# soedinglab/MMseqs2

Hardware: AMD Instinct MI355X
Metric: sw_gcells_per_s (higher is better)
Workload: dtype int16

## Files before the change

mmseqs2_amd/csrc/mmgpu_api.hip:

```cpp
#include <algorithm>
#include <atomic>
#include <thread>
#include <cmath>
#include <cstdio>
#include <cstring>
#include <numeric>
#include <string>
#include <vector>

#include "mmgpu_internal.h"

#include <chrono>

using namespace mmgpu;

namespace mmgpu {
thread_local std::string g_last_error;
}
using mmgpu::g_last_error;

extern "C" const char *mmgpu_last_error(void) { return g_last_error.c_str(); }

extern "C" int mmgpu_init(mmgpu_ctx **out, int device_id) {
    if (!out) return fail(MMGPU_ERR_ARG, "mmgpu_init: ctx is NULL");
// ... 477 lines not shown
        v.len = b->m_len.as<uint32_t>();
        v.n = (uint32_t)b->m_h_len.size();
        v.max_len = b->m_max_len;
        v.h_len = b->m_h_len.data();
    } else {
        v.res = c->db.res;
        v.off4 = c->db.off4;
        v.len = c->db.len;
        v.n = c->db.n;
        v.max_len = c->db.max_len;
        v.h_len = c->h_len.data();
    }
    return v;
}

static void pick_class(uint32_t qlen, int *rows_per_lane, bool *multi) {
    constexpr uint32_t max_rows = 16u * (uint32_t)SW_MAX_R;
    const uint32_t n_tiles = (qlen + max_rows - 1) / max_rows;
    const uint32_t rows = (qlen + n_tiles - 1) / n_tiles;
    *rows_per_lane = (int)std::max<uint32_t>(1u, (rows + 15) / 16);
    *multi = n_tiles > 1;
}

static uint32_t job_slots(uint32_t round, uint64_t rounds) {
    const uint64_t slots = std::max<uint64_t>(1, rounds) * round;
    if (slots >= JOB_ROUND) return (uint32_t)std::min<uint64_t>(JOB_HITS, slots / JOB_ROUND * JOB_ROUND);
    return slots >= 16 ? 16u : round;
}

struct DeviceLists {
    const mmgpu_pf_hit *hits = nullptr;
    const uint32_t *counts = nullptr;
// ... 276 lines not shown
    }
    if (multi && mode >= MMGPU_SW_START)
        add_rev_jobs(i, hit_cursor, pf_stride, shape, (uint64_t)Q.qlen * ((Q.qlen + c->mean_len) / 2 + 1));
    max_tlen = tv.max_len;
}

int SwPrepare::copy_queries() {
    for (uint32_t i = 0; i < nq; i++) {
        const mmgpu_sw_query &Q = qs[i];
        if (Q.qlen == 0) {
            b->h_qout_off[i + 1] = out_cursor;
            continue;
        }
        int qminp;
        if (int e = copy_query(i, &qminp)) return e;
        int rpl; bool multi;
        pick_class(Q.qlen, &rpl, &multi);
        any_multi |= multi;
        const uint32_t shape = (multi ? 32u : 0u) + (uint32_t)rpl - 1;
        const int grp = sw_shape_group(shape);
        const uint32_t held = multi && sw_multi_resident(sw_tiles(Q.qlen, rpl), rpl, par->alphabet, SW_RESIDENT_LDS) ? sw_tiles(Q.qlen, rpl) : 1u;
        b->group_lds[grp] = std::max(b->group_lds[grp], (size_t)held * sw_profile_bytes(rpl, par->alphabet));
        const uint32_t round = (multi && Q.qlen >= LONG_QUERY) ? JOB_ROUND / 4 : JOB_ROUND;
        const uint32_t n_slots = pf ? pf_stride : dense ? dense->count[i] : Q.n_targets;
        if (pf) add_slot_jobs(i, shape, round, multi);
        else deferred.push_back(Deferred{i, hit_cursor, out_cursor, shape, round, multi});
        hit_cursor += n_slots;
        out_cursor += n_slots;
        b->h_qout_off[i + 1] = out_cursor;
    }
    return MMGPU_OK;
}

void SwPrepare::cut_list_jobs_of(size_t from, size_t to) {
    std::vector<uint32_t> ord;
    for (size_t d = from; d < to; d++) {
        const Deferred &D = deferred[d];
        const mmgpu_sw_query &Q = qs[D.query];
// ... 493 lines not shown
            L.out = b->x_out ? b->x_out : b->d_out.as<mmgpu_sw_hit>();
            L.mat = b->d_mat.as<int8_t>();
            L.alphabet = b->alphabet;
            L.gap_open = b->gap_open;
            L.gap_extend = b->gap_extend;
            L.q_hit_count = b->from_pf ? b->d_pf_counts.as<uint32_t>() : nullptr;
            L.hit_stride = b->slot_stride;
            L.scratch = b->d_scratch.as<uint2>();
            L.scratch_cols = b->scratch_cols;
            L.scratch_busy = b->d_scratch_busy.as<uint32_t>();
            L.scratch_slots = std::max<uint32_t>(b->scratch_slots, 1);
            L.resident_lds = SW_RESIDENT_LDS;
            L.rev_mode = rev_only ? 2 : (b->mode == MMGPU_SW_START_NOT_WORD ? 1 : 0);
            L.rev_only = rev_only ? 1 : 0;
            L.rev_force = rev_force;
            HIP_TRY(launch_sw(L, g, b->group_lds[g], b->mode >= MMGPU_SW_START, st));
            if (g == SW_GROUPS - 1 && b->n_rev_jobs && b->mode >= MMGPU_SW_START) {
                SwLaunch Rv = L;
                Rv.jobs = b->d_jobs.as<SwJob>() + b->n_jobs;
                Rv.n_jobs = b->n_rev_jobs;
                HIP_TRY(launch_sw_rev_multi(Rv, b->group_lds[g], st));
            }
            if (getenv("MMGPU_TRACE")) {
                fprintf(stderr, "[sw_run] group %d jobs %u lds %zu both %d from_pf %d scratch_cols %u\n", g, L.n_jobs, b->group_lds[g], (int)(b->mode >= MMGPU_SW_START), (int)b->from_pf, b->scratch_cols);
                fflush(stderr);
                const auto t0 = std::chrono::steady_clock::now();
                hipError_t e = hipStreamSynchronize(st);
                fprintf(stderr, "[sw_run] group %d done after %.2f ms: %s\n", g,
                        std::chrono::duration<double, std::milli>(std::chrono::steady_clock::now() - t0).count(), hipGetErrorString(e));
                fflush(stderr);
// ... 774 lines not shown
```

mmseqs2_amd/csrc/mmgpu_internal.h:

```cpp
#ifndef MMGPU_INTERNAL_H
#define MMGPU_INTERNAL_H

#include <hip/hip_runtime.h>
#include <stdint.h>
#include <cstdlib>
#include <cstring>

#include <algorithm>
#include <array>
#include <string>
#include <map>
#include <mutex>
#include <chrono>
#include <memory>
#include <vector>
#include <thread>
#include <atomic>

#include "../../include/mmgpu.h"
#include "nucl_core.h"
#include "block_plan.h"

namespace mmgpu {

// ... 55 lines not shown
    const uint32_t *hit_out;
    mmgpu_sw_hit *out;
    const int8_t *mat;
    int alphabet;
    int gap_open, gap_extend;
    uint2 *scratch;
    uint32_t scratch_cols;
    uint32_t *scratch_busy;
    uint32_t scratch_slots;
    uint32_t resident_lds = 0;
    const uint32_t *q_hit_count;
    uint32_t hit_stride;
    int rev_mode = 0;
    int rev_only = 0;
    const uint8_t *rev_force = nullptr;
};

constexpr int SW_PF_MAX_LIST = 16384;
constexpr int SW_FROM_PF_STAT_SLOTS = 64;

struct SwFromPfArgs {
    const mmgpu_pf_hit *pf_hits;
    uint32_t pf_stride;
    const uint32_t *hit_count;
    uint32_t stride;
    const uint32_t *q_off;
    const uint32_t *t_len;
    uint32_t *hit_target, *hit_out;
    unsigned long long *cells, *pairs;
    uint32_t *count_copy;
// ... 21 lines not shown
static_assert(SW_GROUPS == 3 || SW_GROUPS == 4, "three or four kernel groups");
int sw_shape_group(uint32_t shape);
hipError_t launch_sw(const SwLaunch &L, int group, size_t lds_bytes, bool both_passes, hipStream_t stream);
#ifndef MMGPU_SW_HALF
#define MMGPU_SW_HALF 1
#endif
bool launch_sw_half(const SwLaunch &L, int group, size_t lds_bytes, bool both_passes, hipStream_t stream);
void warm_sw_half();

constexpr int SW_LDS_HEADER = SW_REV_JOB_MAX * 2 + 64;
__host__ __device__ constexpr int lane_stride_bytes(int R) {
    int slots = (R * 2 + 15) / 16;
    if ((slots & 1) == 0) slots += 1;
    return slots * 16;
}
__host__ __device__ constexpr uint32_t sw_profile_bytes(int R, int alphabet) {
    return (uint32_t)(alphabet + 1) * 16u * (uint32_t)lane_stride_bytes(R);
}
#ifndef MMGPU_SW_RESIDENT_LDS
#define MMGPU_SW_RESIDENT_LDS 65536
#endif
constexpr uint32_t SW_RESIDENT_LDS = MMGPU_SW_RESIDENT_LDS;
static_assert(SW_RESIDENT_LDS <= 65536u, "a workgroup asks for at most 64 KB of dynamic LDS");
__host__ __device__ constexpr uint32_t sw_tiles(uint32_t qlen, int R) { return (qlen + 16u * (uint32_t)R - 1u) / (16u * (uint32_t)R); }
__host__ __device__ constexpr bool sw_multi_resident(uint32_t n_tiles, int R, int alphabet, uint32_t budget) {
    return (unsigned long long)n_tiles * sw_profile_bytes(R, alphabet) + (unsigned long long)SW_LDS_HEADER <= (unsigned long long)budget;
}
static_assert(sw_multi_resident(2, 28, 21, 65536) && sw_multi_resident(3, 24, 21, 65536) && !sw_multi_resident(3, 25, 21, 65536) &&
              !sw_multi_resident(4, 22, 21, 65536) && !sw_multi_resident(2, 8, 21, 0), "residency rule");

constexpr int SCAN_CLASSES = 5;
constexpr int SCAN_MULTI = SCAN_CLASSES - 1;
constexpr int SCAN_MAX_R = 32;
constexpr int SCAN_ROUND = 32;
constexpr int SCAN_JOB_TARGETS = 16 * SCAN_ROUND;
__host__ __device__ constexpr int scan_class_rows(int cls) { return cls == 0 ? 8 : cls == 1 ? 16 : cls == 2 ? 24 : 32; }
__host__ __device__ constexpr uint32_t scan_cols(uint32_t len, int R) { return (len + (uint32_t)R - 1u) / (uint32_t)R * (uint32_t)R; }
__host__ __device__ constexpr uint32_t scan_park_row_words(uint32_t longest) { return 2u * ((scan_cols(longest, SCAN_MAX_R) + 1u + 15u) & ~15u); }

constexpr uint64_t SCAN_NO_PROFILE = ~0ull;

struct ScanJob {
    uint32_t query;
    uint32_t begin, end;
// ... 868 lines not shown
```

mmseqs2_amd/csrc/sw_body.h:

```cpp
#pragma once
#include "mmgpu_internal.h"
#include "pf_device.h"

namespace mmgpu {

namespace {

constexpr int GROUP = 16;
constexpr int WAVES = 4;
constexpr int GROUPS_PER_WAVE = 64 / GROUP;
constexpr int HITS_PER_WAVE = 2 * GROUPS_PER_WAVE;
constexpr unsigned NEG2 = 0x80008000u;

typedef short s16x2 __attribute__((ext_vector_type(2)));
typedef unsigned short u16x2 __attribute__((ext_vector_type(2)));

__device__ __forceinline__ unsigned pk_add_sat(unsigned a, unsigned b) {
    return __builtin_bit_cast(unsigned, __builtin_elementwise_add_sat(__builtin_bit_cast(s16x2, a),
                                                                      __builtin_bit_cast(s16x2, b)));
}
__device__ __forceinline__ unsigned pk_max_s(unsigned a, unsigned b) {
    return __builtin_bit_cast(unsigned, __builtin_elementwise_max(__builtin_bit_cast(s16x2, a),
                                                                  __builtin_bit_cast(s16x2, b)));
}
// ... 13 lines not shown
constexpr int SW_HALF_MAX_GAP = 2048;
constexpr int SW_HALF_MARK = -1;
typedef _Float16 h16x2 __attribute__((ext_vector_type(2)));
__device__ __forceinline__ h16x2 as_h(unsigned a) { return __builtin_bit_cast(h16x2, a); }
__device__ __forceinline__ unsigned as_u(h16x2 a) { return __builtin_bit_cast(unsigned, a); }
__device__ __forceinline__ unsigned h_add(unsigned a, unsigned b) { return as_u(as_h(a) + as_h(b)); }
__device__ __forceinline__ unsigned h_sub(unsigned a, unsigned b) { return as_u(as_h(a) - as_h(b)); }
__device__ __forceinline__ unsigned h_max(unsigned a, unsigned b) {
    return as_u(__builtin_elementwise_maximum(as_h(a), as_h(b)));
}
__device__ __forceinline__ unsigned h_max3(unsigned a, unsigned b, unsigned c) {
    return as_u(__builtin_elementwise_maximum(__builtin_elementwise_maximum(as_h(a), as_h(b)), as_h(c)));
}
__device__ __forceinline__ unsigned short h_bits(int v) { return __builtin_bit_cast(unsigned short, (_Float16)v); }
__device__ __forceinline__ int h_value(unsigned bits) { return (int)(float)__builtin_bit_cast(_Float16, (unsigned short)bits); }
__device__ __forceinline__ unsigned from_lane_above(unsigned head, unsigned v) {
    return __builtin_amdgcn_update_dpp(head, v, 0x111 , 0xF, 0xF, false);
}
__device__ __forceinline__ unsigned from_lane_above_or_zero(unsigned v) {
    return __builtin_amdgcn_update_dpp(0u, v, 0x111 , 0xF, 0xF, true);
}

#ifndef MMGPU_SW_PREFETCH
#define MMGPU_SW_PREFETCH 1
#endif
#define SW_KEEP_IN_ROW(x) asm volatile("" : "+v"(x))

template <int R>
struct Tile {
    static constexpr int ROWS = GROUP * R;
    static constexpr int LANE_STRIDE = lane_stride_bytes(R);
    static constexpr int ROW_STRIDE = GROUP * LANE_STRIDE;
};
static_assert(GROUP == 16, "sw_profile_bytes and sw_tiles (mmgpu_internal.h) assume 16-lane groups");

template <int R, bool REV, bool HALF = false>
__device__ __forceinline__ void build_profile(unsigned char *lds, const uint8_t *q, const int8_t *cb, int qlen,
                                              int tile_base, const int8_t *mat, int alphabet, const int8_t *prof) {
    using T = Tile<R>;
    const int total = (alphabet + 1) * T::ROWS;
    for (int idx = threadIdx.x; idx < total; idx += blockDim.x) {
        const int letter = idx / T::ROWS;
        const int row = idx - letter * T::ROWS;
        const int rg = tile_base + row;
        short v = (short)-32768;
        if (letter < alphabet && rg < qlen) {
            const int qi = REV ? (qlen - 1 - rg) : rg;
            v = prof ? (short)prof[letter * qlen + qi] : (short)((int)mat[letter * alphabet + q[qi]] + (int)cb[qi]);
        }
        const int lane = row / R, r = row - lane * R;
        if constexpr (HALF) v = (short)h_bits(v);
        *reinterpret_cast<short *>(lds + letter * T::ROW_STRIDE + lane * T::LANE_STRIDE + r * 2) = v;
    }
}
// ... 2 lines not shown
    const mmgpu_sw_hit &f = L.out[slot];
    const int s = f.score;
    if (L.rev_mode == 2) return s > 0 && L.rev_force[slot] != 0;
    return s > 0 && s >= min_start && !(L.rev_mode == 1 && f.word != 0);
}

constexpr int SW_REV_JOB_HITS = 1024;
static_assert(SW_REV_JOB_HITS == SW_REV_JOB_MAX, "host and kernel disagree on the reverse job size");
static_assert(SW_LDS_HEADER == SW_REV_JOB_HITS * 2 + 64, "the header holds the live hits and the scheduling words");
constexpr int SW_HALF_FLAG_AT = SW_REV_JOB_HITS * 2 + 20;
__device__ __forceinline__ uint32_t sw_half_any_marked() {
    extern __shared__ __attribute__((aligned(16))) unsigned char lds_all[];
    return *reinterpret_cast<const uint32_t *>(lds_all + SW_HALF_FLAG_AT);
}

template <int R, bool MULTI, bool REV, bool PF, bool HALF = false, bool MARKED = false>
__device__ __forceinline__ void sw_body(const SwLaunch &L, const SwJob job) {
    static_assert(!(HALF || MARKED) || (!MULTI && !REV && !(HALF && MARKED)), "f16 and its int16 re-run: single-tile forward scans");
    constexpr bool PACKED = REV || MARKED;
    using T = Tile<R>;
    extern __shared__ __attribute__((aligned(16))) unsigned char lds_all[];
    uint16_t *live = reinterpret_cast<uint16_t *>(lds_all);
    uint32_t *live_wave = reinterpret_cast<uint32_t *>(lds_all + SW_REV_JOB_HITS * 2);
    uint32_t *next_chunk = reinterpret_cast<uint32_t *>(lds_all + SW_REV_JOB_HITS * 2 + 16);
    uint32_t *half_flag = reinterpret_cast<uint32_t *>(lds_all + SW_HALF_FLAG_AT);
    unsigned char *lds = lds_all + SW_LDS_HEADER;
    if (MULTI) __builtin_amdgcn_s_setprio(3);
    const int lane = threadIdx.x & 63;
    const int wave = __builtin_amdgcn_readfirstlane(threadIdx.x >> 6);
    const int g = lane & (GROUP - 1);
    const int grp = lane / GROUP;

    const uint32_t qbeg = L.q_off[job.query];
    const int qlen = (int)(L.q_off[job.query + 1] - qbeg);
    const uint8_t *q = L.q_res + qbeg;
    const int8_t *cb = L.q_cb + qbeg;
    const int qbias = L.q_bias[job.query];
    const int8_t *prof = nullptr;
    if (L.q_prof_off) {
        const uint32_t po = L.q_prof_off[job.query];
        if (po != 0xFFFFFFFFu) prof = L.q_prof + po;
    }
    const int n_tiles = MULTI ? (int)sw_tiles((uint32_t)qlen, R) : 1;
    const uint32_t tile_bytes = sw_profile_bytes(R, L.alphabet);
    const bool resident = MULTI && sw_multi_resident((uint32_t)n_tiles, R, L.alphabet, L.resident_lds);
    const bool dynamic = !MULTI || resident;
    auto build_all_tiles = [&]() {
        for (int tile = 0; tile < n_tiles; ++tile)
            build_profile<R, REV>(lds + (uint32_t)tile * tile_bytes, q, cb, qlen, tile * T::ROWS, L.mat, L.alphabet, prof);
        __syncthreads();
    };

    const unsigned go2 = (HALF ? (unsigned)h_bits(L.gap_open) : (unsigned)L.gap_open) * 0x10001u;
    const unsigned ge2 = (HALF ? (unsigned)h_bits(L.gap_extend) : (unsigned)L.gap_extend) * 0x10001u;
    const unsigned pad_letter = (unsigned)L.alphabet;

    if (threadIdx.x == 0) *next_chunk = 0;
    if (HALF && threadIdx.x == 0) *half_flag = 0;
    if (!MULTI && !PACKED) {
        build_profile<R, REV, HALF>(lds, q, cb, qlen, 0, L.mat, L.alphabet, prof);
        __syncthreads();
    }
    if (MULTI && !REV && resident) build_all_tiles();

    uint32_t n_hits = job.hit_end - job.hit_begin;
    if (PACKED) {
        const int min_start = REV ? L.q_minstart[job.query] : 0;
        uint32_t total = 0;
        for (uint32_t base = 0; base < n_hits; base += WAVES * 64) {
            const uint32_t idx = base + threadIdx.x;
            bool pass = false;
            if (idx < n_hits) {
                const uint32_t slot = L.hit_out[job.hit_begin + idx];
                pass = MARKED ? L.out[slot].score == SW_HALF_MARK : sw_rev_wanted(L, slot, min_start);
            }
// ... 2 lines not shown
            __syncthreads();
            uint32_t before = 0, round_total = 0;
#pragma unroll
            for (int w = 0; w < WAVES; ++w) {
                const uint32_t c = live_wave[w];
                before += w < wave ? c : 0u;
                round_total += c;
            }
            if (pass) live[total + before + (uint32_t)__popcll(bal & ((1ull << lane) - 1ull))] = (uint16_t)idx;
            total += round_total;
            __syncthreads();
        }
        n_hits = total;
        if (n_hits == 0) return;
        if (!MULTI) {
            build_profile<R, REV>(lds, q, cb, qlen, 0, L.mat, L.alphabet, prof);
            __syncthreads();
        }
        if (MULTI && resident) build_all_tiles();
    }
    const uint32_t n_iter = (n_hits + WAVES * HITS_PER_WAVE - 1) / (WAVES * HITS_PER_WAVE);

    for (uint32_t it = 0; dynamic || it < n_iter; ++it) {
        uint32_t chunk = it * WAVES + wave;
        if (dynamic) {
            if (lane == 0) chunk = atomicAdd(next_chunk, 1u);
            chunk = __builtin_amdgcn_readfirstlane(chunk);
        }
        const uint32_t slot0 = chunk * HITS_PER_WAVE;
        if (dynamic && slot0 >= n_hits) break;

// ... 14 lines not shown
            fb = fa;
            if (vA) fa = L.out[L.hit_out[hA]];
            if (vB) fb = L.out[L.hit_out[hB]];
            colsA = vA ? fa.t_end + 1 : 0;
            colsB = vB ? fb.t_end + 1 : 0;
            endA = colsA > 0 ? fa.t_end : 0;
            endB = colsB > 0 ? fb.t_end : 0;
            r0A = colsA > 0 ? qlen - 1 - fa.q_end : 0;
            r0B = colsB > 0 ? qlen - 1 - fb.q_end : 0;
            rev_target = (colsA > 0 ? (unsigned)fa.score & 0xFFFFu : 0xFFFFu) | ((colsB > 0 ? (unsigned)fb.score & 0xFFFFu : 0xFFFFu) << 16);
        }
        int ncols = colsA > colsB ? colsA : colsB;
        ncols = max(ncols, __shfl_xor(ncols, 16));
        ncols = max(ncols, __shfl_xor(ncols, 32));
        ncols = __builtin_amdgcn_readfirstlane(ncols);
        const int nsteps = ncols + GROUP - 1;
        int mincols = colsA < colsB ? colsA : colsB;
        mincols = min(mincols, __shfl_xor(mincols, 16));
        mincols = min(mincols, __shfl_xor(mincols, 32));
        mincols = __builtin_amdgcn_readfirstlane(mincols);

        unsigned long long bestA = 0, bestB = 0;

        uint2 *scr = nullptr;
        unsigned scr_grp = 0;
        if (MULTI) {
            scr = L.scratch + (size_t)((job.shape >> 8) * WAVES + wave) * GROUPS_PER_WAVE * 2 * L.scratch_cols;
            scr_grp = (unsigned)grp * 2u * L.scratch_cols;
        }

        for (int tile = 0; tile < n_tiles; ++tile) {
// ... 83 lines not shown
                    b = bfi(mb, b, pad4);
                }
                const unsigned lo = __builtin_amdgcn_perm(b, a, REV ? 0x06020703u : 0x05010400u);
                const unsigned hi = __builtin_amdgcn_perm(b, a, REV ? 0x04000501u : 0x07030602u);
                lq = ((unsigned long long)hi << 32) | lo;
            };
            auto head_letters = [&](int c, int j) -> unsigned {
                if (LETTER_BLOCKS && LETTER_QUEUE) { const unsigned v = (unsigned)lq; lq >>= 16; return v; }
                if (LETTER_BLOCKS) return (unsigned)(lq >> (16 * j));
                const unsigned sh = (unsigned)(REV ? 3 - j : j) * 8u;
                const unsigned la0 = __builtin_amdgcn_ubfe(wA, sh, 8u);
                const unsigned lb0 = __builtin_amdgcn_ubfe(wB, sh, 8u);
                return (c < colsA ? la0 : pad_letter) | ((c < colsB ? lb0 : pad_letter) << 8);
            };
            letter_block(0);
            let = from_lane_above(head_letters(0, 0), let);
            if (PF) load_rows(let, pav_next, pbv_next);

            for (int s0 = -1; s0 < nsteps; s0 += 4) {
            if (MULTI && s0 > 0 && ((s0 + 1) & 15) == 0) {
                bnd = bnd_next;
                if (has_above) bnd_next = boundary16(((s0 + 1) >> 4) + 1);
            }
            const int jn = min(4, nsteps - s0);
#pragma nounroll
            for (int j = s0 < 0 ? 1 : 0; j < jn; ++j) {
                const int s = s0 + j;
                if (has_below && s >= GROUP) {
                    if (g == GROUP - 1) (scr_out + (s - GROUP))[scr_grp] = make_uint2(out_H, out_F);
                }
                const unsigned Hup = MULTI ? from_lane_above(bnd.x, out_H) : from_lane_above_or_zero(out_H);
                unsigned f = MULTI ? from_lane_above(bnd.y, out_F) : from_lane_above_or_zero(out_F);
                if (MULTI) {
                    bnd.x = __builtin_amdgcn_update_dpp(bnd.x, bnd.x, 0x12F, 0xF, 0xF, false);
                    bnd.y = __builtin_amdgcn_update_dpp(bnd.y, bnd.y, 0x12F, 0xF, 0xF, false);
                }
                unsigned pav[ND], pbv[ND];
                if (PF) {
#pragma unroll
                    for (int k = 0; k < ND; ++k) { pav[k] = pav_next[k]; pbv[k] = pbv_next[k]; }
                } else {
                    load_rows(let, pav, pbv);
                }

                unsigned hd = Hup_prev;
                Hup_prev = Hup;
                unsigned cmax = 0;
                unsigned pre[R], es[R];
#pragma unroll
                for (int r = 0; r < R; ++r) {
                    unsigned P = __builtin_amdgcn_perm(pbv[r / 2], pav[r / 2], (r & 1) ? 0x07060302u : 0x05040100u);
                    if (REV) P = __builtin_amdgcn_bitop3_b32(aux[r], P, NEG2, 0xCA);
                    if constexpr (HALF) {
                        pre[r] = h_add(r == 0 ? hd : Hp[r - 1], P);
                        es[r] = h_sub(E[r], ge2);
                    } else {
                        pre[r] = pk_max_s(pk_add_sat(r == 0 ? hd : Hp[r - 1], P), E[r]);
                        es[r] = pk_sub_sat_u(E[r], ge2);
                    }
                }
                let = from_lane_above(head_letters(s + 1, j), let);
                if (PF) load_rows(let, pav_next, pbv_next);
#pragma unroll
                for (int r = 0; r < R; ++r) {
                    unsigned h;
                    if constexpr (HALF) {
                        h = h_max3(pre[r], E[r], f);
                        const unsigned fs = h_sub(f, ge2);
                        const unsigned t = h_sub(h, go2);
                        cmax = r == 0 ? h : h_max(cmax, h);
                        f = h_max3(fs, t, 0u);
                        E[r] = h_max3(es[r], t, 0u);
                    } else {
                        h = pk_max_s(pre[r], f);
                        const unsigned fs = pk_sub_sat_u(f, ge2);
                        const unsigned t = pk_sub_sat_u(h, go2);
// ... 49 lines not shown
            if (!REV) {
#pragma unroll
                for (int r = R - 1; r >= 0; --r) {
                    if ((aux[r] & 0xFFFFu) == sA) rowA_first = (unsigned)r;
                    if ((aux[r] >> 16) == sB) rowB_first = (unsigned)r;
                }
            } else {
                sA = sA == (rev_target & 0xFFFFu) ? sA : 0u;
                sB = sB == (rev_target >> 16) ? sB : 0u;
            }
            const unsigned rgA = (unsigned)(tile_base + g * R) + rowA_first;
            const unsigned rgB = (unsigned)(tile_base + g * R) + rowB_first;
            unsigned long long keyA = sA ? ((unsigned long long)sA << 32) | ((0xFFFFu - (bestcol & 0xFFFFu)) << 16) | (0xFFFFu - rgA) : 0ull;
            unsigned long long keyB = sB ? ((unsigned long long)sB << 32) | ((0xFFFFu - (bestcol >> 16)) << 16) | (0xFFFFu - rgB) : 0ull;
#pragma unroll
            for (int m = 1; m < GROUP; m <<= 1) {
                const unsigned long long oa = __shfl_xor(keyA, m), ob = __shfl_xor(keyB, m);
                keyA = oa > keyA ? oa : keyA;
                keyB = ob > keyB ? ob : keyB;
            }
            bestA = keyA > bestA ? keyA : bestA;
            bestB = keyB > bestB ? keyB : bestB;
        }

        if (g == 0) {
#pragma unroll
            for (int half = 0; half < 2; ++half) {
                const bool valid = half ? vB : vA;
                if (!valid) continue;
                const unsigned long long key = half ? bestB : bestA;
                const uint32_t h = half ? hB : hA;
// ... 13 lines not shown
                    *o = res;
                    if (marked) *half_flag = 1;
                } else {
                    const int end = half ? endB : endA;
                    const int cols = half ? colsB : colsA;
                    if (cols > 0) {
                        o->t_start = (score == o->score) ? end - col : -2;
                        o->q_start = (score == o->score) ? qlen - 1 - row : -2;
                    }
                }
            }
        }
    }
}

template <int R, bool MULTI, bool BOTH>
__device__ __forceinline__ void sw_passes(const SwLaunch &L, const SwJob &job) {
    if constexpr (R <= SW_MAX_R) {
        constexpr bool PF = MMGPU_SW_PREFETCH && !MULTI && (BOTH || R <= 24);
        if (!(BOTH && L.rev_only)) sw_body<R, MULTI, false, PF>(L, job);
        if constexpr (BOTH && !MULTI) {
            __threadfence_block();
            __syncthreads();
            sw_body<R, MULTI, true, PF>(L, job);
        }
    }
}

#ifndef MMGPU_SW_WAVES_G0F
#define MMGPU_SW_WAVES_G0F 4
#endif
#ifndef MMGPU_SW_WAVES_G0B
#define MMGPU_SW_WAVES_G0B 2
#endif
#ifndef MMGPU_SW_WAVES_G1F
#define MMGPU_SW_WAVES_G1F 3
#endif
#ifndef MMGPU_SW_WAVES_G1B
#define MMGPU_SW_WAVES_G1B 2
// ... 6 lines not shown
```

mmseqs2_amd/csrc/sw_half_kernel.hip:

```cpp
#include "mmgpu_internal.h"
#include "pf_device.h"
#include "sw_body.h"

namespace mmgpu {

namespace {

template <int R, bool BOTH>
__device__ __forceinline__ void sw_half_passes(const SwLaunch &L, const SwJob &job) {
    if constexpr (R <= SW_MAX_R) {
        constexpr bool PF = MMGPU_SW_PREFETCH && (BOTH || R <= 24);
        sw_body<R, false, false, PF, true, false>(L, job);
        __threadfence_block();
        __syncthreads();
        if (sw_half_any_marked()) {
            sw_body<R, false, false, PF, false, true>(L, job);
            __threadfence_block();
            __syncthreads();
        }
        if constexpr (BOTH) sw_body<R, false, true, PF>(L, job);
    }
}

constexpr bool SW_HALF_FORWARD_ONLY[3] = {false, false, false};

template <int G, bool BOTH>
__global__ __launch_bounds__(WAVES * 64)
__attribute__((amdgpu_waves_per_eu(G == 0 ? (BOTH ? MMGPU_SW_WAVES_G0B : MMGPU_SW_WAVES_G0F)
                                           : (G == 1 ? (BOTH ? MMGPU_SW_WAVES_G1B : MMGPU_SW_WAVES_G1F) : SW_MIN_WAVES),
                                   G == 1 && BOTH ? MMGPU_SW_WAVES_G1B : 8))) void sw_half_kernel(SwLaunch L) {
    SwJob job = L.jobs[blockIdx.x];
    if (L.q_hit_count) {
        const uint32_t lim = job.query * L.hit_stride + L.q_hit_count[job.query];
        job.hit_end = job.hit_end < lim ? job.hit_end : lim;
        if (job.hit_end <= job.hit_begin) return;
    }
#define MMGPU_SW_SINGLE(R) case (R) - 1: sw_half_passes<R, BOTH>(L, job); break;
    if constexpr (G == 0) {
        switch (job.shape & 0xFFu) {
            MMGPU_SW_SINGLE(1) MMGPU_SW_SINGLE(2) MMGPU_SW_SINGLE(3) MMGPU_SW_SINGLE(4) MMGPU_SW_SINGLE(5) MMGPU_SW_SINGLE(6)
            MMGPU_SW_SINGLE(7) MMGPU_SW_SINGLE(8) MMGPU_SW_SINGLE(9) MMGPU_SW_SINGLE(10) MMGPU_SW_SINGLE(11) MMGPU_SW_SINGLE(12)
            default: break;
        }
    } else if constexpr (G == 1) {
        switch (job.shape & 0xFFu) {
            MMGPU_SW_SINGLE(13) MMGPU_SW_SINGLE(14) MMGPU_SW_SINGLE(15) MMGPU_SW_SINGLE(16) MMGPU_SW_SINGLE(17) MMGPU_SW_SINGLE(18)
            MMGPU_SW_SINGLE(19) MMGPU_SW_SINGLE(20) MMGPU_SW_SINGLE(21) MMGPU_SW_SINGLE(22) MMGPU_SW_SINGLE(23) MMGPU_SW_SINGLE(24)
            default: break;
        }
    } else {
        switch (job.shape & 0xFFu) {
            MMGPU_SW_SINGLE(25) MMGPU_SW_SINGLE(26) MMGPU_SW_SINGLE(27) MMGPU_SW_SINGLE(28) MMGPU_SW_SINGLE(29) MMGPU_SW_SINGLE(30)
            MMGPU_SW_SINGLE(31) MMGPU_SW_SINGLE(32)
            default: break;
        }
    }
#undef MMGPU_SW_SINGLE
}

#ifdef MMGPU_SW_HALF_AUDIT_FORWARD
template __global__ void sw_half_kernel<0, false>(SwLaunch);
template __global__ void sw_half_kernel<1, false>(SwLaunch);
template __global__ void sw_half_kernel<2, false>(SwLaunch);
#endif

}

bool launch_sw_half(const SwLaunch &L, int group, size_t lds_bytes, bool both_passes, hipStream_t stream) {
    if (group < 0 || group > 2 || (group == 2 && SW_GROUPS != 4)) return false;
    if (!both_passes && !SW_HALF_FORWARD_ONLY[group]) return false;
    dim3 grid(L.n_jobs), block(WAVES * 64);
    const size_t lds = lds_bytes + SW_LDS_HEADER;
// ... 15 lines not shown
```

mmseqs2_amd/csrc/sw_kernel.hip:

```cpp
#include "mmgpu_internal.h"
#include "pf_device.h"
#include "sw_body.h"

namespace mmgpu {

namespace {

#define MMGPU_SW_MULTI_ALL                                                                                                          \
    MMGPU_SW_MULTI(8) MMGPU_SW_MULTI(9) MMGPU_SW_MULTI(10) MMGPU_SW_MULTI(11) MMGPU_SW_MULTI(12) MMGPU_SW_MULTI(13) MMGPU_SW_MULTI(14) \
    MMGPU_SW_MULTI(15) MMGPU_SW_MULTI(16) MMGPU_SW_MULTI(17) MMGPU_SW_MULTI(18) MMGPU_SW_MULTI(19) MMGPU_SW_MULTI(20) MMGPU_SW_MULTI(21) \
    MMGPU_SW_MULTI(22) MMGPU_SW_MULTI(23) MMGPU_SW_MULTI(24) MMGPU_SW_MULTI(25) MMGPU_SW_MULTI(26) MMGPU_SW_MULTI(27) MMGPU_SW_MULTI(28) \
    MMGPU_SW_MULTI(29) MMGPU_SW_MULTI(30) MMGPU_SW_MULTI(31) MMGPU_SW_MULTI(32)
template <int G, bool BOTH>
__global__ __launch_bounds__(WAVES * 64)
__attribute__((amdgpu_waves_per_eu(G == 0 ? (BOTH ? MMGPU_SW_WAVES_G0B : MMGPU_SW_WAVES_G0F)
                                           : (G == 1 ? (BOTH ? MMGPU_SW_WAVES_G1B : MMGPU_SW_WAVES_G1F) : SW_MIN_WAVES),
                                   G == 1 && BOTH ? MMGPU_SW_WAVES_G1B : 8))) void sw_kernel(SwLaunch L) {
    SwJob job = L.jobs[blockIdx.x];
    if (L.q_hit_count) {
        const uint32_t lim = job.query * L.hit_stride + L.q_hit_count[job.query];
        job.hit_end = job.hit_end < lim ? job.hit_end : lim;
        if (job.hit_end <= job.hit_begin) return;
    }
    __shared__ uint32_t scratch_slot;
    const bool claims = G == SW_GROUPS - 1 && (job.shape & 0xFFu) >= 32u;
    if (claims) {
        if (threadIdx.x == 0) {
            uint32_t s = blockIdx.x % L.scratch_slots;
            while (atomicCAS(&L.scratch_busy[s], 0u, 1u) != 0u) s = s + 1 == L.scratch_slots ? 0u : s + 1;
            scratch_slot = s;
        }
        __syncthreads();
        job.shape = (job.shape & 0xFFu) | (scratch_slot << 8);
    }
#define MMGPU_SW_SINGLE(R) case (R) - 1: sw_passes<R, false, BOTH>(L, job); break;
#define MMGPU_SW_MULTI(R) case 32 + (R) - 1: sw_passes<R, true, BOTH>(L, job); break;
    if constexpr (G == 0) {
        switch (job.shape & 0xFFu) {
            MMGPU_SW_SINGLE(1) MMGPU_SW_SINGLE(2) MMGPU_SW_SINGLE(3) MMGPU_SW_SINGLE(4) MMGPU_SW_SINGLE(5) MMGPU_SW_SINGLE(6)
            MMGPU_SW_SINGLE(7) MMGPU_SW_SINGLE(8) MMGPU_SW_SINGLE(9) MMGPU_SW_SINGLE(10) MMGPU_SW_SINGLE(11) MMGPU_SW_SINGLE(12)
            default: break;
        }
    } else if constexpr (G == 1) {
        switch (job.shape & 0xFFu) {
            MMGPU_SW_SINGLE(13) MMGPU_SW_SINGLE(14) MMGPU_SW_SINGLE(15) MMGPU_SW_SINGLE(16) MMGPU_SW_SINGLE(17) MMGPU_SW_SINGLE(18)
            MMGPU_SW_SINGLE(19) MMGPU_SW_SINGLE(20) MMGPU_SW_SINGLE(21) MMGPU_SW_SINGLE(22) MMGPU_SW_SINGLE(23) MMGPU_SW_SINGLE(24)
            default: break;
        }
    } else if constexpr (SW_GROUPS == 4 && G == 2) {
        switch (job.shape & 0xFFu) {
            MMGPU_SW_SINGLE(25) MMGPU_SW_SINGLE(26) MMGPU_SW_SINGLE(27) MMGPU_SW_SINGLE(28) MMGPU_SW_SINGLE(29) MMGPU_SW_SINGLE(30)
            MMGPU_SW_SINGLE(31) MMGPU_SW_SINGLE(32)
            default: break;
        }
    } else if constexpr (SW_GROUPS == 4) {
        switch (job.shape & 0xFFu) {
            MMGPU_SW_MULTI_ALL
            default: break;
        }
    } else {
        switch (job.shape & 0xFFu) {
            MMGPU_SW_SINGLE(25) MMGPU_SW_SINGLE(26) MMGPU_SW_SINGLE(27) MMGPU_SW_SINGLE(28) MMGPU_SW_SINGLE(29) MMGPU_SW_SINGLE(30)
            MMGPU_SW_SINGLE(31) MMGPU_SW_SINGLE(32)
            MMGPU_SW_MULTI_ALL
            default: break;
        }
    }
#undef MMGPU_SW_SINGLE
#undef MMGPU_SW_MULTI
#undef MMGPU_SW_MULTI_ALL
    if (claims) {
        __syncthreads();
        if (threadIdx.x == 0) {
            __threadfence();
            atomicExch(&L.scratch_busy[scratch_slot], 0u);
        }
    }
}

__global__ __launch_bounds__(WAVES * 64) __attribute__((amdgpu_waves_per_eu(SW_MIN_WAVES))) void sw_rev_multi_kernel(SwLaunch L) {
    SwJob job = L.jobs[blockIdx.x];
    if (L.q_hit_count) {
        const uint32_t lim = job.query * L.hit_stride + L.q_hit_count[job.query];
        job.hit_end = job.hit_end < lim ? job.hit_end : lim;
        if (job.hit_end <= job.hit_begin) return;
// ... 100 lines not shown
        int rev = 0;
        if (hipOccupancyMaxActiveBlocksPerMultiprocessor(&rev, sw_rev_multi_kernel, WAVES * 64, lds) == hipSuccess) per_cu = std::max(per_cu, rev);
    }
    if (e != hipSuccess || per_cu < 1) per_cu = 8;
    per_cu = per_cu + 1 > 8 ? 8 : per_cu + 1;
    return (uint32_t)per_cu * (uint32_t)(compute_units > 0 ? compute_units : 256);
}

hipError_t launch_sw_rev_multi(const SwLaunch &L, size_t lds_bytes, hipStream_t stream) {
    if (L.n_jobs == 0) return hipSuccess;
    hipLaunchKernelGGL(sw_rev_multi_kernel, dim3(L.n_jobs), dim3(WAVES * 64), lds_bytes + SW_LDS_HEADER, stream, L);
    return hipGetLastError();
}

int sw_shape_group(uint32_t shape) {
    if (shape >= 32) return SW_GROUPS - 1;
    const int R = (int)shape + 1;
    return R <= 12 ? 0 : (R <= 24 ? 1 : 2);
}

static bool sw_half_eligible(const SwLaunch &L) {
    return MMGPU_SW_HALF && !L.rev_only && L.gap_open >= 0 && L.gap_open <= SW_HALF_MAX_GAP && L.gap_extend >= 0 &&
           L.gap_extend <= SW_HALF_MAX_GAP;
}

hipError_t launch_sw(const SwLaunch &L, int group, size_t lds_bytes, bool both_passes, hipStream_t stream) {
    static_assert(GROUP == 16, "the shape codes assume 16-lane groups");
    if (L.n_jobs == 0) return hipSuccess;
    if (sw_half_eligible(L) && launch_sw_half(L, group, lds_bytes, both_passes, stream)) return hipGetLastError();
    dim3 grid(L.n_jobs), block(WAVES * 64);
    const size_t lds = lds_bytes + SW_LDS_HEADER;
    switch (group * 2 + (both_passes ? 1 : 0)) {
        case 0: hipLaunchKernelGGL((sw_kernel<0, false>), grid, block, lds, stream, L); break;
        case 1: hipLaunchKernelGGL((sw_kernel<0, true>), grid, block, lds, stream, L); break;
        case 2: hipLaunchKernelGGL((sw_kernel<1, false>), grid, block, lds, stream, L); break;
        case 3: hipLaunchKernelGGL((sw_kernel<1, true>), grid, block, lds, stream, L); break;
        case 4: hipLaunchKernelGGL((sw_kernel<2, false>), grid, block, lds, stream, L); break;
        case 5: hipLaunchKernelGGL((sw_kernel<2, true>), grid, block, lds, stream, L); break;
        case 6: hipLaunchKernelGGL((sw_kernel<SW_GROUPS - 1, false>), grid, block, lds, stream, L); break;
        case 7: hipLaunchKernelGGL((sw_kernel<SW_GROUPS - 1, true>), grid, block, lds, stream, L); break;
        default: return hipErrorInvalidValue;
    }
// ... 11 lines not shown
```

Baseline: 4913.

## Add 32-lane wide single-tile SW shape for queries up to twice max tile

Queries longer than one 16-lane tile but at most twice that length now go to a new wide shape. It uses 32-lane groups spanning two DPP rows, so the whole query sits in one tile. This avoids the multi-tile path with its scratch boundary exchange, scratch slot claiming and repeated passes over targets. The cost is an extra cross-row DPP per lane shift, twice the profile LDS, half the hits per wave, and a smaller job round. A half-precision path is also wired in behind an env switch.

```diff
diff --git a/mmseqs2_amd/csrc/mmgpu_api.hip b/mmseqs2_amd/csrc/mmgpu_api.hip
--- a/mmseqs2_amd/csrc/mmgpu_api.hip
+++ b/mmseqs2_amd/csrc/mmgpu_api.hip
@@ -515,8 +515,14 @@
     return v;
 }
 
-static void pick_class(uint32_t qlen, int *rows_per_lane, bool *multi) {
+static void pick_class(uint32_t qlen, int *rows_per_lane, bool *multi, bool *wide) {
     constexpr uint32_t max_rows = 16u * (uint32_t)SW_MAX_R;
+    *wide = mmgpu::sw_wide_enabled() && qlen > max_rows && qlen <= 2 * max_rows;
+    if (*wide) {
+        *rows_per_lane = (int)((qlen + 31) / 32);
+        *multi = false;
+        return;
+    }
     const uint32_t n_tiles = (qlen + max_rows - 1) / max_rows;
     const uint32_t rows = (qlen + n_tiles - 1) / n_tiles;
     *rows_per_lane = (int)std::max<uint32_t>(1u, (rows + 15) / 16);
@@ -823,14 +829,14 @@
         }
         int qminp;
         if (int e = copy_query(i, &qminp)) return e;
-        int rpl; bool multi;
-        pick_class(Q.qlen, &rpl, &multi);
+        int rpl; bool multi, wide;
+        pick_class(Q.qlen, &rpl, &multi, &wide);
         any_multi |= multi;
-        const uint32_t shape = (multi ? 32u : 0u) + (uint32_t)rpl - 1;
+        const uint32_t shape = (multi ? SW_SHAPE_MULTI : wide ? SW_SHAPE_WIDE : 0u) + (uint32_t)rpl - 1;
         const int grp = sw_shape_group(shape);
         const uint32_t held = multi && sw_multi_resident(sw_tiles(Q.qlen, rpl), rpl, par->alphabet, SW_RESIDENT_LDS) ? sw_tiles(Q.qlen, rpl) : 1u;
-        b->group_lds[grp] = std::max(b->group_lds[grp], (size_t)held * sw_profile_bytes(rpl, par->alphabet));
-        const uint32_t round = (multi && Q.qlen >= LONG_QUERY) ? JOB_ROUND / 4 : JOB_ROUND;
+        b->group_lds[grp] = std::max(b->group_lds[grp], (size_t)held * sw_profile_bytes(rpl, par->alphabet, wide ? 32 : 16));
+        const uint32_t round = (multi && Q.qlen >= LONG_QUERY) ? JOB_ROUND / 4 : wide ? JOB_ROUND / 2 : JOB_ROUND;
         const uint32_t n_slots = pf ? pf_stride : dense ? dense->count[i] : Q.n_targets;
         if (pf) add_slot_jobs(i, shape, round, multi);
         else deferred.push_back(Deferred{i, hit_cursor, out_cursor, shape, round, multi});
@@ -1354,6 +1360,7 @@
             L.rev_mode = rev_only ? 2 : (b->mode == MMGPU_SW_START_NOT_WORD ? 1 : 0);
             L.rev_only = rev_only ? 1 : 0;
             L.rev_force = rev_force;
+            L.half_wide = sw_half_wide() ? 1 : 0;
             HIP_TRY(launch_sw(L, g, b->group_lds[g], b->mode >= MMGPU_SW_START, st));
             if (g == SW_GROUPS - 1 && b->n_rev_jobs && b->mode >= MMGPU_SW_START) {
                 SwLaunch Rv = L;
diff --git a/mmseqs2_amd/csrc/mmgpu_internal.h b/mmseqs2_amd/csrc/mmgpu_internal.h
--- a/mmseqs2_amd/csrc/mmgpu_internal.h
+++ b/mmseqs2_amd/csrc/mmgpu_internal.h
@@ -93,6 +93,7 @@
     int rev_mode = 0;
     int rev_only = 0;
     const uint8_t *rev_force = nullptr;
+    int half_wide = 1;
 };
 
 constexpr int SW_PF_MAX_LIST = 16384;
@@ -144,8 +145,8 @@
     if ((slots & 1) == 0) slots += 1;
     return slots * 16;
 }
-__host__ __device__ constexpr uint32_t sw_profile_bytes(int R, int alphabet) {
-    return (uint32_t)(alphabet + 1) * 16u * (uint32_t)lane_stride_bytes(R);
+__host__ __device__ constexpr uint32_t sw_profile_bytes(int R, int alphabet, int lanes = 16) {
+    return (uint32_t)(alphabet + 1) * (uint32_t)lanes * (uint32_t)lane_stride_bytes(R);
 }
 #ifndef MMGPU_SW_RESIDENT_LDS
 #define MMGPU_SW_RESIDENT_LDS 65536
@@ -158,6 +159,14 @@
 }
 static_assert(sw_multi_resident(2, 28, 21, 65536) && sw_multi_resident(3, 24, 21, 65536) && !sw_multi_resident(3, 25, 21, 65536) &&
               !sw_multi_resident(4, 22, 21, 65536) && !sw_multi_resident(2, 8, 21, 0), "residency rule");
+
+constexpr uint32_t SW_SHAPE_MULTI = 32, SW_SHAPE_WIDE = 64;
+constexpr int SW_WIDE_MIN_R = (16 * SW_MAX_R + 1 + 31) / 32;
+static_assert(sw_profile_bytes(SW_MAX_R, 21, 32) == 2 * sw_profile_bytes(SW_MAX_R, 21) &&
+              sw_profile_bytes(SW_MAX_R, 21, 32) + SW_LDS_HEADER <= 65536u, "a wide tile fits a workgroup's 64 KB");
+static_assert((lane_stride_bytes(SW_MAX_R) / 16) % 2 == 1 && (lane_stride_bytes(SW_WIDE_MIN_R) / 16) % 2 == 1, "odd number of 16-byte slots");
+bool sw_wide_enabled();
+bool sw_half_wide();
 
 constexpr int SCAN_CLASSES = 5;
 constexpr int SCAN_MULTI = SCAN_CLASSES - 1;
diff --git a/mmseqs2_amd/csrc/sw_body.h b/mmseqs2_amd/csrc/sw_body.h
--- a/mmseqs2_amd/csrc/sw_body.h
+++ b/mmseqs2_amd/csrc/sw_body.h
@@ -51,11 +51,19 @@
 }
 __device__ __forceinline__ unsigned short h_bits(int v) { return __builtin_bit_cast(unsigned short, (_Float16)v); }
 __device__ __forceinline__ int h_value(unsigned bits) { return (int)(float)__builtin_bit_cast(_Float16, (unsigned short)bits); }
+template <int W>
+__device__ __forceinline__ unsigned across_rows(unsigned x, unsigned v) {
+    static_assert(W == 16 || W == 32, "groups of one or two DPP rows");
+    if constexpr (W == 32) x = __builtin_amdgcn_update_dpp(x, v, 0x138 , 0xA, 0x1, false);
+    return x;
+}
+template <int W = GROUP>
 __device__ __forceinline__ unsigned from_lane_above(unsigned head, unsigned v) {
-    return __builtin_amdgcn_update_dpp(head, v, 0x111 , 0xF, 0xF, false);
-}
+    return across_rows<W>(__builtin_amdgcn_update_dpp(head, v, 0x111 , 0xF, 0xF, false), v);
+}
+template <int W = GROUP>
 __device__ __forceinline__ unsigned from_lane_above_or_zero(unsigned v) {
-    return __builtin_amdgcn_update_dpp(0u, v, 0x111 , 0xF, 0xF, true);
+    return across_rows<W>(__builtin_amdgcn_update_dpp(0u, v, 0x111 , 0xF, 0xF, true), v);
 }
 
 #ifndef MMGPU_SW_PREFETCH
@@ -63,18 +71,18 @@
 #endif
 #define SW_KEEP_IN_ROW(x) asm volatile("" : "+v"(x))
 
-template <int R>
+template <int R, int W = GROUP>
 struct Tile {
-    static constexpr int ROWS = GROUP * R;
+    static constexpr int ROWS = W * R;
     static constexpr int LANE_STRIDE = lane_stride_bytes(R);
-    static constexpr int ROW_STRIDE = GROUP * LANE_STRIDE;
+    static constexpr int ROW_STRIDE = W * LANE_STRIDE;
 };
-static_assert(GROUP == 16, "sw_profile_bytes and sw_tiles (mmgpu_internal.h) assume 16-lane groups");
-
-template <int R, bool REV, bool HALF = false>
+static_assert(GROUP == 16, "sw_profile_bytes' default and sw_tiles (mmgpu_internal.h) assume 16-lane groups for all but the wide shapes");
+
+template <int R, bool REV, bool HALF = false, int W = GROUP>
 __device__ __forceinline__ void build_profile(unsigned char *lds, const uint8_t *q, const int8_t *cb, int qlen,
                                               int tile_base, const int8_t *mat, int alphabet, const int8_t *prof) {
-    using T = Tile<R>;
+    using T = Tile<R, W>;
     const int total = (alphabet + 1) * T::ROWS;
     for (int idx = threadIdx.x; idx < total; idx += blockDim.x) {
         const int letter = idx / T::ROWS;
@@ -107,11 +115,13 @@
     return *reinterpret_cast<const uint32_t *>(lds_all + SW_HALF_FLAG_AT);
 }
 
-template <int R, bool MULTI, bool REV, bool PF, bool HALF = false, bool MARKED = false>
+template <int R, bool MULTI, bool REV, bool PF, bool HALF = false, bool MARKED = false, int W = GROUP>
 __device__ __forceinline__ void sw_body(const SwLaunch &L, const SwJob job) {
     static_assert(!(HALF || MARKED) || (!MULTI && !REV && !(HALF && MARKED)), "f16 and its int16 re-run: single-tile forward scans");
+    static_assert(W == GROUP || (W == 2 * GROUP && !MULTI), "the boundary row of a multi-tile body rotates inside one DPP row");
     constexpr bool PACKED = REV || MARKED;
-    using T = Tile<R>;
+    constexpr int HITS_PER_WAVE = 2 * 64 / W;
+    using T = Tile<R, W>;
     extern __shared__ __attribute__((aligned(16))) unsigned char lds_all[];
     uint16_t *live = reinterpret_cast<uint16_t *>(lds_all);
     uint32_t *live_wave = reinterpret_cast<uint32_t *>(lds_all + SW_REV_JOB_HITS * 2);
@@ -121,8 +131,8 @@
     if (MULTI) __builtin_amdgcn_s_setprio(3);
     const int lane = threadIdx.x & 63;
     const int wave = __builtin_amdgcn_readfirstlane(threadIdx.x >> 6);
-    const int g = lane & (GROUP - 1);
-    const int grp = lane / GROUP;
+    const int g = lane & (W - 1);
+    const int grp = lane / W;
 
     const uint32_t qbeg = L.q_off[job.query];
     const int qlen = (int)(L.q_off[job.query + 1] - qbeg);
@@ -151,7 +161,7 @@
     if (threadIdx.x == 0) *next_chunk = 0;
     if (HALF && threadIdx.x == 0) *half_flag = 0;
     if (!MULTI && !PACKED) {
-        build_profile<R, REV, HALF>(lds, q, cb, qlen, 0, L.mat, L.alphabet, prof);
+        build_profile<R, REV, HALF, W>(lds, q, cb, qlen, 0, L.mat, L.alphabet, prof);
         __syncthreads();
     }
     if (MULTI && !REV && resident) build_all_tiles();
@@ -184,7 +194,7 @@
         n_hits = total;
         if (n_hits == 0) return;
         if (!MULTI) {
-            build_profile<R, REV>(lds, q, cb, qlen, 0, L.mat, L.alphabet, prof);
+            build_profile<R, REV, false, W>(lds, q, cb, qlen, 0, L.mat, L.alphabet, prof);
             __syncthreads();
         }
         if (MULTI && resident) build_all_tiles();
@@ -229,7 +239,7 @@
         ncols = max(ncols, __shfl_xor(ncols, 16));
         ncols = max(ncols, __shfl_xor(ncols, 32));
         ncols = __builtin_amdgcn_readfirstlane(ncols);
-        const int nsteps = ncols + GROUP - 1;
+        const int nsteps = ncols + W - 1;
         int mincols = colsA < colsB ? colsA : colsB;
         mincols = min(mincols, __shfl_xor(mincols, 16));
         mincols = min(mincols, __shfl_xor(mincols, 32));
@@ -343,7 +353,7 @@
                 return (c < colsA ? la0 : pad_letter) | ((c < colsB ? lb0 : pad_letter) << 8);
             };
             letter_block(0);
-            let = from_lane_above(head_letters(0, 0), let);
+            let = from_lane_above<W>(head_letters(0, 0), let);
             if (PF) load_rows(let, pav_next, pbv_next);
 
             for (int s0 = -1; s0 < nsteps; s0 += 4) {
@@ -358,8 +368,8 @@
                 if (has_below && s >= GROUP) {
                     if (g == GROUP - 1) (scr_out + (s - GROUP))[scr_grp] = make_uint2(out_H, out_F);
                 }
-                const unsigned Hup = MULTI ? from_lane_above(bnd.x, out_H) : from_lane_above_or_zero(out_H);
-                unsigned f = MULTI ? from_lane_above(bnd.y, out_F) : from_lane_above_or_zero(out_F);
+                const unsigned Hup = MULTI ? from_lane_above<W>(bnd.x, out_H) : from_lane_above_or_zero<W>(out_H);
+                unsigned f = MULTI ? from_lane_above<W>(bnd.y, out_F) : from_lane_above_or_zero<W>(out_F);
                 if (MULTI) {
                     bnd.x = __builtin_amdgcn_update_dpp(bnd.x, bnd.x, 0x12F, 0xF, 0xF, false);
                     bnd.y = __builtin_amdgcn_update_dpp(bnd.y, bnd.y, 0x12F, 0xF, 0xF, false);
@@ -388,7 +398,7 @@
                         es[r] = pk_sub_sat_u(E[r], ge2);
                     }
                 }
-                let = from_lane_above(head_letters(s + 1, j), let);
+                let = from_lane_above<W>(head_letters(s + 1, j), let);
                 if (PF) load_rows(let, pav_next, pbv_next);
 #pragma unroll
                 for (int r = 0; r < R; ++r) {
@@ -468,7 +478,7 @@
             unsigned long long keyA = sA ? ((unsigned long long)sA << 32) | ((0xFFFFu - (bestcol & 0xFFFFu)) << 16) | (0xFFFFu - rgA) : 0ull;
             unsigned long long keyB = sB ? ((unsigned long long)sB << 32) | ((0xFFFFu - (bestcol >> 16)) << 16) | (0xFFFFu - rgB) : 0ull;
 #pragma unroll
-            for (int m = 1; m < GROUP; m <<= 1) {
+            for (int m = 1; m < W; m <<= 1) {
                 const unsigned long long oa = __shfl_xor(keyA, m), ob = __shfl_xor(keyB, m);
                 keyA = oa > keyA ? oa : keyA;
                 keyB = ob > keyB ? ob : keyB;
@@ -512,15 +522,15 @@
     }
 }
 
-template <int R, bool MULTI, bool BOTH>
+template <int R, bool MULTI, bool BOTH, int W = GROUP>
 __device__ __forceinline__ void sw_passes(const SwLaunch &L, const SwJob &job) {
-    if constexpr (R <= SW_MAX_R) {
+    if constexpr (R <= SW_MAX_R && (W == GROUP || R >= SW_WIDE_MIN_R)) {
         constexpr bool PF = MMGPU_SW_PREFETCH && !MULTI && (BOTH || R <= 24);
-        if (!(BOTH && L.rev_only)) sw_body<R, MULTI, false, PF>(L, job);
+        if (!(BOTH && L.rev_only)) sw_body<R, MULTI, false, PF, false, false, W>(L, job);
         if constexpr (BOTH && !MULTI) {
             __threadfence_block();
             __syncthreads();
-            sw_body<R, MULTI, true, PF>(L, job);
+            sw_body<R, MULTI, true, PF, false, false, W>(L, job);
         }
     }
 }
diff --git a/mmseqs2_amd/csrc/sw_half_kernel.hip b/mmseqs2_amd/csrc/sw_half_kernel.hip
--- a/mmseqs2_amd/csrc/sw_half_kernel.hip
+++ b/mmseqs2_amd/csrc/sw_half_kernel.hip
@@ -6,19 +6,24 @@
 
 namespace {
 
-template <int R, bool BOTH>
+template <int R, bool BOTH, int W = GROUP>
 __device__ __forceinline__ void sw_half_passes(const SwLaunch &L, const SwJob &job) {
-    if constexpr (R <= SW_MAX_R) {
+    if constexpr (R <= SW_MAX_R && (W == GROUP || R >= SW_WIDE_MIN_R)) {
         constexpr bool PF = MMGPU_SW_PREFETCH && (BOTH || R <= 24);
-        sw_body<R, false, false, PF, true, false>(L, job);
+        const bool f16 = W == GROUP || L.half_wide;
+        if (f16) {
+            sw_body<R, false, false, PF, true, false, W>(L, job);
+        } else {
+            for (uint32_t h = job.hit_begin + threadIdx.x; h < job.hit_end; h += blockDim.x) L.out[L.hit_out[h]].score = SW_HALF_MARK;
+        }
         __threadfence_block();
         __syncthreads();
-        if (sw_half_any_marked()) {
-            sw_body<R, false, false, PF, false, true>(L, job);
+        if (!f16 || sw_half_any_marked()) {
+            sw_body<R, false, false, PF, false, true, W>(L, job);
             __threadfence_block();
             __syncthreads();
         }
-        if constexpr (BOTH) sw_body<R, false, true, PF>(L, job);
+        if constexpr (BOTH) sw_body<R, false, true, PF, false, false, W>(L, job);
     }
 }
 
@@ -36,6 +41,7 @@
         if (job.hit_end <= job.hit_begin) return;
     }
 #define MMGPU_SW_SINGLE(R) case (R) - 1: sw_half_passes<R, BOTH>(L, job); break;
+#define MMGPU_SW_WIDE(R) case 64 + (R) - 1: sw_half_passes<R, BOTH, 2 * GROUP>(L, job); break;
     if constexpr (G == 0) {
         switch (job.shape & 0xFFu) {
             MMGPU_SW_SINGLE(1) MMGPU_SW_SINGLE(2) MMGPU_SW_SINGLE(3) MMGPU_SW_SINGLE(4) MMGPU_SW_SINGLE(5) MMGPU_SW_SINGLE(6)
@@ -46,16 +52,22 @@
         switch (job.shape & 0xFFu) {
             MMGPU_SW_SINGLE(13) MMGPU_SW_SINGLE(14) MMGPU_SW_SINGLE(15) MMGPU_SW_SINGLE(16) MMGPU_SW_SINGLE(17) MMGPU_SW_SINGLE(18)
             MMGPU_SW_SINGLE(19) MMGPU_SW_SINGLE(20) MMGPU_SW_SINGLE(21) MMGPU_SW_SINGLE(22) MMGPU_SW_SINGLE(23) MMGPU_SW_SINGLE(24)
+            MMGPU_SW_WIDE(8) MMGPU_SW_WIDE(9) MMGPU_SW_WIDE(10) MMGPU_SW_WIDE(11) MMGPU_SW_WIDE(12) MMGPU_SW_WIDE(13) MMGPU_SW_WIDE(14)
+            MMGPU_SW_WIDE(15) MMGPU_SW_WIDE(16) MMGPU_SW_WIDE(17) MMGPU_SW_WIDE(18) MMGPU_SW_WIDE(19) MMGPU_SW_WIDE(20) MMGPU_SW_WIDE(21)
+            MMGPU_SW_WIDE(22) MMGPU_SW_WIDE(23) MMGPU_SW_WIDE(24)
             default: break;
         }
     } else {
         switch (job.shape & 0xFFu) {
             MMGPU_SW_SINGLE(25) MMGPU_SW_SINGLE(26) MMGPU_SW_SINGLE(27) MMGPU_SW_SINGLE(28) MMGPU_SW_SINGLE(29) MMGPU_SW_SINGLE(30)
             MMGPU_SW_SINGLE(31) MMGPU_SW_SINGLE(32)
+            MMGPU_SW_WIDE(25) MMGPU_SW_WIDE(26) MMGPU_SW_WIDE(27) MMGPU_SW_WIDE(28) MMGPU_SW_WIDE(29) MMGPU_SW_WIDE(30) MMGPU_SW_WIDE(31)
+            MMGPU_SW_WIDE(32)
             default: break;
         }
     }
 #undef MMGPU_SW_SINGLE
+#undef MMGPU_SW_WIDE
 }
 
 #ifdef MMGPU_SW_HALF_AUDIT_FORWARD
diff --git a/mmseqs2_amd/csrc/sw_kernel.hip b/mmseqs2_amd/csrc/sw_kernel.hip
--- a/mmseqs2_amd/csrc/sw_kernel.hip
+++ b/mmseqs2_amd/csrc/sw_kernel.hip
@@ -23,7 +23,7 @@
         if (job.hit_end <= job.hit_begin) return;
     }
     __shared__ uint32_t scratch_slot;
-    const bool claims = G == SW_GROUPS - 1 && (job.shape & 0xFFu) >= 32u;
+    const bool claims = G == SW_GROUPS - 1 && (job.shape & 0xFFu) >= SW_SHAPE_MULTI && (job.shape & 0xFFu) < SW_SHAPE_WIDE;
     if (claims) {
         if (threadIdx.x == 0) {
             uint32_t s = blockIdx.x % L.scratch_slots;
@@ -35,6 +35,12 @@
     }
 #define MMGPU_SW_SINGLE(R) case (R) - 1: sw_passes<R, false, BOTH>(L, job); break;
 #define MMGPU_SW_MULTI(R) case 32 + (R) - 1: sw_passes<R, true, BOTH>(L, job); break;
+#define MMGPU_SW_WIDE(R) case 64 + (R) - 1: sw_passes<R, false, BOTH, 2 * GROUP>(L, job); break;
+#define MMGPU_SW_WIDE_M MMGPU_SW_WIDE(8) MMGPU_SW_WIDE(9) MMGPU_SW_WIDE(10) MMGPU_SW_WIDE(11) MMGPU_SW_WIDE(12) MMGPU_SW_WIDE(13)                \
+    MMGPU_SW_WIDE(14) MMGPU_SW_WIDE(15) MMGPU_SW_WIDE(16) MMGPU_SW_WIDE(17) MMGPU_SW_WIDE(18) MMGPU_SW_WIDE(19) MMGPU_SW_WIDE(20)               \
+    MMGPU_SW_WIDE(21) MMGPU_SW_WIDE(22) MMGPU_SW_WIDE(23) MMGPU_SW_WIDE(24)
+#define MMGPU_SW_WIDE_L MMGPU_SW_WIDE(25) MMGPU_SW_WIDE(26) MMGPU_SW_WIDE(27) MMGPU_SW_WIDE(28) MMGPU_SW_WIDE(29) MMGPU_SW_WIDE(30)            \
+    MMGPU_SW_WIDE(31) MMGPU_SW_WIDE(32)
     if constexpr (G == 0) {
         switch (job.shape & 0xFFu) {
             MMGPU_SW_SINGLE(1) MMGPU_SW_SINGLE(2) MMGPU_SW_SINGLE(3) MMGPU_SW_SINGLE(4) MMGPU_SW_SINGLE(5) MMGPU_SW_SINGLE(6)
@@ -45,12 +51,14 @@
         switch (job.shape & 0xFFu) {
             MMGPU_SW_SINGLE(13) MMGPU_SW_SINGLE(14) MMGPU_SW_SINGLE(15) MMGPU_SW_SINGLE(16) MMGPU_SW_SINGLE(17) MMGPU_SW_SINGLE(18)
             MMGPU_SW_SINGLE(19) MMGPU_SW_SINGLE(20) MMGPU_SW_SINGLE(21) MMGPU_SW_SINGLE(22) MMGPU_SW_SINGLE(23) MMGPU_SW_SINGLE(24)
+            MMGPU_SW_WIDE_M
             default: break;
         }
     } else if constexpr (SW_GROUPS == 4 && G == 2) {
         switch (job.shape & 0xFFu) {
             MMGPU_SW_SINGLE(25) MMGPU_SW_SINGLE(26) MMGPU_SW_SINGLE(27) MMGPU_SW_SINGLE(28) MMGPU_SW_SINGLE(29) MMGPU_SW_SINGLE(30)
             MMGPU_SW_SINGLE(31) MMGPU_SW_SINGLE(32)
+            MMGPU_SW_WIDE_L
             default: break;
         }
     } else if constexpr (SW_GROUPS == 4) {
@@ -62,6 +70,7 @@
         switch (job.shape & 0xFFu) {
             MMGPU_SW_SINGLE(25) MMGPU_SW_SINGLE(26) MMGPU_SW_SINGLE(27) MMGPU_SW_SINGLE(28) MMGPU_SW_SINGLE(29) MMGPU_SW_SINGLE(30)
             MMGPU_SW_SINGLE(31) MMGPU_SW_SINGLE(32)
+            MMGPU_SW_WIDE_L
             MMGPU_SW_MULTI_ALL
             default: break;
         }
@@ -69,6 +78,9 @@
 #undef MMGPU_SW_SINGLE
 #undef MMGPU_SW_MULTI
 #undef MMGPU_SW_MULTI_ALL
+#undef MMGPU_SW_WIDE
+#undef MMGPU_SW_WIDE_M
+#undef MMGPU_SW_WIDE_L
     if (claims) {
         __syncthreads();
         if (threadIdx.x == 0) {
@@ -199,9 +211,23 @@
 }
 
 int sw_shape_group(uint32_t shape) {
-    if (shape >= 32) return SW_GROUPS - 1;
+    if (shape >= SW_SHAPE_WIDE) return (int)(shape - SW_SHAPE_WIDE) + 1 <= 24 ? 1 : 2;
+    if (shape >= SW_SHAPE_MULTI) return SW_GROUPS - 1;
     const int R = (int)shape + 1;
     return R <= 12 ? 0 : (R <= 24 ? 1 : 2);
+}
+
+static bool env_switch(const char *name, bool unset) {
+    const char *v = getenv(name);
+    return v && *v ? atoi(v) != 0 : unset;
+}
+bool sw_wide_enabled() {
+    static const bool on = env_switch("MMGPU_SW_WIDE", true);
+    return on;
+}
+bool sw_half_wide() {
+    static const bool on = env_switch("MMGPU_SW_HALF_WIDE", true);
+    return on;
 }
 
 static bool sw_half_eligible(const SwLaunch &L) {
@@ -210,7 +236,7 @@
 }
 
 hipError_t launch_sw(const SwLaunch &L, int group, size_t lds_bytes, bool both_passes, hipStream_t stream) {
-    static_assert(GROUP == 16, "the shape codes assume 16-lane groups");
+    static_assert(GROUP == 16 && SW_SHAPE_MULTI == 32 && SW_SHAPE_WIDE == 64, "the shape codes of the dispatch: 16-lane groups, + 32 multi-tile, + 64 wide");
     if (L.n_jobs == 0) return hipSuccess;
     if (sw_half_eligible(L) && launch_sw_half(L, group, lds_bytes, both_passes, stream)) return hipGetLastError();
     dim3 grid(L.n_jobs), block(WAVES * 64);
```

New measurement: 5001, median of 6. 1.02x the previous value.
